# oppo-us-research/PoP-Net

Measured on AMD Instinct MI355X. Metric: depth-frames/sec end-to-end (480x640), higher is better.
Workload: dtype bf16

## Files before the change

popnet_amd/csrc/api.hip:

```cpp
#pragma clang fp contract(off)
#include <cmath>
#include <cstdarg>
#include <cstdio>
#include <cstdlib>
#include <cstring>
#include "pn_internal.h"
#include "preproc_pixel.h"

template <typename TIN>
__global__ void preprocess_kernel(const TIN *__restrict__ depth, float *__restrict__ out, int B, int H, int W, int S,
                                  double scale_x, double scale_y, float dmax, float mean, float stdv) {
    const unsigned pix = blockIdx.x * blockDim.x + threadIdx.x;
    if (pix >= (unsigned)(S * S)) return;
    const int b = blockIdx.y;
    const int dy = (int)(pix / (unsigned)S);
    const int dx = (int)(pix - (unsigned)dy * (unsigned)S);
    const size_t gid = (size_t)b * S * S + pix;

    out[gid] = pn_preproc_pixel(depth + (size_t)b * H * W, H, W, dy, dx, scale_x, scale_y, dmax, mean, stdv);
}

PnSwitches pn_read_switches() {
    auto set = [](const char *name) { return getenv(name) != nullptr; };
    auto num = [](const char *name, int unset) { const char *e = getenv(name); return e ? atoi(e) : unset; };
    auto is = [](const char *name, const char *value) { const char *e = getenv(name); return e && !strcmp(e, value); };
    PnSwitches s;
    s.no_conv3 = set("POPNET_NO_CONV3");
    s.conv3_rpg8 = set("POPNET_CONV3_RPG8");
    s.conv3_pt14 = num("POPNET_CONV3_PT14", 0);
    s.conv3_nbuf2 = set("POPNET_CONV3_NBUF2");
    s.generic_c64_off = num("POPNET_GENERIC_C64", 1) == 0;
    if (set("POPNET_CONV4")) s.conv4 = num("POPNET_CONV4", 0) == 0 ? 0 : 1;
    s.no_mix = set("POPNET_NO_MIX");
    s.no_bblock = set("POPNET_NO_BBLOCK");
    s.bblock_x3 = num("POPNET_BBLOCK_X3", 0) != 0;
    s.bb64_static = set("POPNET_BB64_STATIC");
    s.bb64_halves = num("POPNET_BB64_HALVES", 1) == 2 ? 2 : 1;
    if (set("POPNET_BB64_STRIP")) { const int v = num("POPNET_BB64_STRIP", 0); s.bb64_strip = v == 1 || v == 2 ? v : 0; }
    s.no_tailfuse = set("POPNET_NO_TAILFUSE");
    s.no_poolfuse = set("POPNET_NO_POOLFUSE");
    s.no_stempool = set("POPNET_NO_STEMPOOL");
    s.no_embed3 = set("POPNET_NO_EMBED3");
    s.train_x3_wide = set("POPNET_TRAIN_X3_WIDE");
    s.train_wgrad_novec = set("POPNET_TRAIN_WGRAD_NOVEC");
    s.trainx_one_stream = num("POPNET_TRAINX_STREAMS", 0) == 1;
    s.trainx_stem_handover = set("POPNET_TRAINX_STEM_HANDOVER");
    s.trainx_stem_gather = is("POPNET_TRAINX_STEM_FWD", "gather");
    s.trainx_stem_bn_separate = is("POPNET_TRAINX_STEM_BN", "separate");
    s.trainx_stem_depth = num("POPNET_TRAINX_STEM_DEPTH", 2);
    s.trainx_pack_gather = is("POPNET_TRAINX_PACK", "gather");
    s.trainx_legacy_wgrad = is("POPNET_TRAINX_WGRAD", "legacy");
    return s;
}

extern "C" {

int pn_abi_version(void) { return PN_ABI_VERSION; }
int pn_build_experiments(void) { return 0; }

pn_ctx *pn_create(int device_id) {
    pn_ctx *ctx = new pn_ctx();
    ctx->device = device_id;
    int ndev = 0;
    hipError_t e = hipGetDeviceCount(&ndev);
    if (e != hipSuccess || device_id < 0 || device_id >= ndev) {
        char buf[256];
        snprintf(buf, sizeof buf, "pn_create: device %d not available (%d devices, %s)", device_id, ndev,
                 hipGetErrorString(e));
        ctx->err = buf;
        ctx->device = -1;
        return ctx;
    }
    hipDeviceProp_t prop;
    if (hipGetDeviceProperties(&prop, device_id) == hipSuccess) ctx->num_cus = prop.multiProcessorCount;
    return ctx;
}

void pn_destroy(pn_ctx *ctx) {
    if (!ctx) return;
    if (ctx->parse_ws) (void)hipFree(ctx->parse_ws);
    pn_parse_big_free(ctx);
    if (ctx->train_ws) (void)hipFree(ctx->train_ws);
    for (void *p : ctx->train_ws_retired) (void)hipFree(p);
    for (auto &e : ctx->train_packs) (void)hipFree(e.buf);
    if (ctx->train_pack_table) (void)hipFree(ctx->train_pack_table);
    delete ctx;
}

}

int pn_set_error(pn_ctx *ctx, int code, const char *fmt, ...) {
    char buf[1024];
    va_list ap;
    va_start(ap, fmt);
    vsnprintf(buf, sizeof(buf), fmt, ap);
    va_end(ap);
    if (ctx) ctx->err = buf;
    return code;
}

extern "C" {

int pn_last_error(pn_ctx *ctx, char *buf, size_t buf_len) {
    if (!ctx) return 0;
    if (buf && buf_len) {
        size_t n = ctx->err.size() < buf_len - 1 ? ctx->err.size() : buf_len - 1;
        memcpy(buf, ctx->err.data(), n);
        buf[n] = 0;
    }
    return (int)ctx->err.size();
}

int pn_preprocess(pn_ctx *ctx, const void *depth_dev, int depth_dtype, int B, int H, int W, float *out_dev, int S,
                  float depth_max, float depth_mean, float depth_std, void *hip_stream) {
    if (!ctx) return PN_ERR_INVALID;
    if (ctx->device < 0) return pn_set_error(ctx, PN_ERR_STATE, "context has no device");
    if (!depth_dev || !out_dev || B < 1 || H < 2 || W < 2 || S < 1)
        return pn_set_error(ctx, PN_ERR_INVALID, "pn_preprocess: bad arguments");
    if (W == 2 * S && H == 2 * S)
        return pn_set_error(ctx, PN_ERR_UNSUPPORTED, "pn_preprocess: %dx%d -> %d is an exact 2x decimation, where cv2.resize(INTER_LINEAR) runs INTER_AREA instead: not built", W, H, S);
    const double inv_x = (double)S / (double)W, inv_y = (double)S / (double)H;
    const double scale_x = 1.0 / inv_x, scale_y = 1.0 / inv_y;
    if (B > 65535 || (size_t)S * S > 0x7fffffffu) return pn_set_error(ctx, PN_ERR_INVALID, "pn_preprocess: batch or output size out of range");
    dim3 grid((unsigned)(((size_t)S * S + 255) / 256), (unsigned)B), block(256);
    hipStream_t s = (hipStream_t)hip_stream;
    if (depth_dtype == PN_DEPTH_F16)
        hipLaunchKernelGGL(preprocess_kernel<_Float16>, grid, block, 0, s, (const _Float16 *)depth_dev, out_dev, B, H, W, S,
                           scale_x, scale_y, depth_max, depth_mean, depth_std);
    else if (depth_dtype == PN_DEPTH_F32)
        hipLaunchKernelGGL(preprocess_kernel<float>, grid, block, 0, s, (const float *)depth_dev, out_dev, B, H, W, S,
                           scale_x, scale_y, depth_max, depth_mean, depth_std);
    else
        return pn_set_error(ctx, PN_ERR_INVALID, "pn_preprocess: unknown depth dtype %d", depth_dtype);
    PN_HIP_CHECK(ctx, hipGetLastError());
    return PN_OK;
}

size_t pn_sizeof_parse_cfg(void) { return sizeof(pn_parse_cfg); }

void pn_parse_cfg_default(pn_parse_cfg *cfg) {
    if (!cfg) return;
    cfg->thresh_heatmap = 0.1f;
    cfg->thresh_paf = 0.05f;
    cfg->num_intermed_pts = 10;
    cfg->downsample = 8;
    cfg->input_size = 224;
    cfg->w_org = 480;
    cfg->h_org = 640;
    cfg->fx = 504.1189880371094;
    cfg->fy = 504.042724609375;
    cfg->cx = 231.7421875;
    cfg->cy = 320.62640380859375;
    cfg->depth_mean = 3.f;
    cfg->depth_std = 2.f;
    cfg->z_readout = PN_Z_READOUT_HEAT_WEIGHTED;
    for (int j = 0; j < PN_NUM_JOINTS; ++j) cfg->z_chn[j] = j;
}

}
```

popnet_amd/csrc/conv_misc.hip:

```cpp
#include "pn_internal.h"
#include "preproc_pixel.h"

typedef __attribute__((ext_vector_type(8))) __bf16 bf16x8;
typedef __attribute__((ext_vector_type(4))) float f32x4;

template <typename T>
__global__ __launch_bounds__(256) void stem7x7_kernel(const float *__restrict__ x, const float *__restrict__ w,
                                                       const float *__restrict__ bias, T *__restrict__ out,
                                                       int H, int W, int Ho, int Wo, int out_cs, int split) {
    __shared__ float tile[37][40];
    __shared__ __attribute__((aligned(16))) float wl[49 * 64];
    const int tid = threadIdx.x;
    const int b = blockIdx.z;
    const int oy0 = blockIdx.y * 16, ox0 = blockIdx.x * 16;
    const int iy0 = oy0 * 2 - 3, ix0 = ox0 * 2 - 3;
    for (int i = tid; i < 49 * 64; i += 256) wl[i] = w[i];
    const float *xb = x + (size_t)b * H * W;
    for (int i = tid; i < 37 * 37; i += 256) {
        int r = i / 37, cc = i - r * 37;
        int iy = iy0 + r, ix = ix0 + cc;
        float v = 0.f;
        if ((unsigned)iy < (unsigned)H && (unsigned)ix < (unsigned)W) v = xb[(size_t)iy * W + ix];
        tile[r][cc] = v;
    }
    __syncthreads();
    const int ty = tid >> 4, tx = tid & 15;
    const int oy = oy0 + ty, ox = ox0 + tx;
    float acc[64];
#pragma unroll
    for (int i = 0; i < 64; ++i) acc[i] = 0.f;
    for (int ky = 0; ky < 7; ++ky) {
#pragma unroll
        for (int kx = 0; kx < 7; ++kx) {
            const float xv = tile[ty * 2 + ky][tx * 2 + kx];
            const f32x4 *wp = reinterpret_cast<const f32x4 *>(&wl[(ky * 7 + kx) * 64]);
#pragma unroll
            for (int i = 0; i < 16; ++i) {
                f32x4 w4 = wp[i];
                acc[4 * i + 0] = fmaf(xv, w4[0], acc[4 * i + 0]);
                acc[4 * i + 1] = fmaf(xv, w4[1], acc[4 * i + 1]);
                acc[4 * i + 2] = fmaf(xv, w4[2], acc[4 * i + 2]);
                acc[4 * i + 3] = fmaf(xv, w4[3], acc[4 * i + 3]);
            }
        }
    }
    if (oy < Ho && ox < Wo) {
        T *op = out + ((size_t)(b * Ho + oy) * Wo + ox) * out_cs;
#pragma unroll
        for (int i = 0; i < 64; ++i) {
            float v = acc[i] + bias[i];
            v = v > 0.f ? v : 0.f;
            const T hi = (T)v;
            op[i] = hi;
            if (split) {
                op[split + i] = (T)(v - (float)hi);
            }
        }
    }
}

typedef __attribute__((ext_vector_type(8))) __bf16 stem_bf16x8;
typedef __attribute__((ext_vector_type(4))) unsigned int stem_u32x4;
#define STEM_PITCH 96

template <bool LO>
__device__ __forceinline__ void stem_put(__bf16 *tile, __bf16 *tile_lo, int idx, float v) {
    const __bf16 vh = (__bf16)v;
    tile[idx] = vh;
    if (LO) tile_lo[idx] = (__bf16)(v - (float)vh);
}
template <int ROWS, bool LO>
__device__ __forceinline__ void stem_fill_f32(__bf16 *tile, __bf16 *tile_lo, const float *xb, int iy0, int ix0, int H, int W, int tid) {
    for (int i = tid; i < ROWS * 38; i += 256) {
        const int r = i / 38, cc = i - r * 38;
        const int iy = iy0 + r, ix = ix0 + cc;
        float v = 0.f;
        if (r < ROWS - 1 && (unsigned)iy < (unsigned)H && (unsigned)ix < (unsigned)W) v = xb[(size_t)iy * W + ix];
        stem_put<LO>(tile, tile_lo, r * STEM_PITCH + cc, v);
    }
}
template <int SRC, int ROWS, bool LO>
__device__ __forceinline__ void stem_fill_frames(__bf16 *tile, __bf16 *tile_lo, const PnFrameSrc &src, int b, int iy0, int ix0, int H, int W, int tid) {
    __shared__ PnAxisX axs[38];
    __shared__ PnAxisY ays[ROWS];
    if (tid < 38) axs[tid] = pn_preproc_axis_x(ix0 + tid, src.scale_x, src.W);
    else if (tid >= 64 && tid < 64 + ROWS) ays[tid - 64] = pn_preproc_axis_y(iy0 + tid - 64, src.scale_y, src.H);
    __syncthreads();
    for (int i = tid; i < ROWS * 38; i += 256) {
        const int r = i / 38, cc = i - r * 38;
        const int iy = iy0 + r, ix = ix0 + cc;
        float v = 0.f;
        if (r < ROWS - 1 && (unsigned)iy < (unsigned)H && (unsigned)ix < (unsigned)W) {
            if (SRC == 1) v = pn_preproc_combine((const _Float16 *)src.frames + (size_t)b * src.H * src.W, src.W, axs[cc], ays[r], src.dmax, src.mean, src.stdv);
            else v = pn_preproc_combine((const float *)src.frames + (size_t)b * src.H * src.W, src.W, axs[cc], ays[r], src.dmax, src.mean, src.stdv);
        }
        stem_put<LO>(tile, tile_lo, r * STEM_PITCH + cc, v);
    }
}
template <bool X3> struct StemW { stem_bf16x8 aw[4][2], awl[X3 ? 4 : 1][2]; float bs[16]; };
template <bool X3>
__device__ __forceinline__ void stem_load_w(StemW<X3> &w, const __bf16 *__restrict__ wfrag, const float *__restrict__ bias, int lane, int q) {
#pragma unroll
    for (int t = 0; t < 4; ++t)
#pragma unroll
        for (int s = 0; s < 2; ++s) {
            w.aw[t][s] = *reinterpret_cast<const stem_bf16x8 *>(wfrag + ((t * 2 + s) * 64 + lane) * 8);
            if (X3) w.awl[t][s] = *reinterpret_cast<const stem_bf16x8 *>(wfrag + ((8 + t * 2 + s) * 64 + lane) * 8);
        }
#pragma unroll
    for (int i = 0; i < 16; ++i) w.bs[i] = bias[16 * q + i];
}
template <bool X3>
__device__ __forceinline__ void stem_row(const StemW<X3> &w, const __bf16 *tile, const __bf16 *tile_lo, int ry, int q, int c, f32x4 (&acc)[4]) {
#pragma unroll
    for (int t = 0; t < 4; ++t) acc[t] = f32x4{0.f, 0.f, 0.f, 0.f};
#pragma unroll
    for (int s = 0; s < 2; ++s) {
        const unsigned *src = reinterpret_cast<const unsigned *>(&tile[(2 * ry + 4 * s + q) * STEM_PITCH + 2 * c]);
        stem_u32x4 raw = {src[0], src[1], src[2], src[3]};
        stem_bf16x8 bf = *reinterpret_cast<stem_bf16x8 *>(&raw);
#pragma unroll
        for (int t = 0; t < 4; ++t) acc[t] = __builtin_amdgcn_mfma_f32_16x16x32_bf16(w.aw[t][s], bf, acc[t], 0, 0, 0);
        if (X3) {
            const unsigned *srl = reinterpret_cast<const unsigned *>(&tile_lo[(2 * ry + 4 * s + q) * STEM_PITCH + 2 * c]);
            stem_u32x4 rawl = {srl[0], srl[1], srl[2], srl[3]};
            stem_bf16x8 bl = *reinterpret_cast<stem_bf16x8 *>(&rawl);
#pragma unroll
            for (int t = 0; t < 4; ++t) {
                acc[t] = __builtin_amdgcn_mfma_f32_16x16x32_bf16(w.aw[t][s], bl, acc[t], 0, 0, 0);
                acc[t] = __builtin_amdgcn_mfma_f32_16x16x32_bf16(w.awl[t][s], bf, acc[t], 0, 0, 0);
            }
        }
    }
}
__device__ __forceinline__ void stem_out16(const f32x4 (&acc)[4], const float (&bs)[16], bool lo, __bf16 (&o)[16]) {
#pragma unroll
    for (int t = 0; t < 4; ++t)
#pragma unroll
        for (int r = 0; r < 4; ++r) {
            float v = acc[t][r] + bs[4 * t + r];
            v = v > 0.f ? v : 0.f;
            const __bf16 hi = (__bf16)v;
            o[4 * t + r] = lo ? (__bf16)(v - (float)hi) : hi;
        }
}

template <bool X3, int SRC = 0>
__global__ __launch_bounds__(256) void stem7x7_mfma_kernel(const float *__restrict__ x, const __bf16 *__restrict__ wfrag,
                                                            const float *__restrict__ bias, __bf16 *__restrict__ out,
                                                            int H, int W, int Ho, int Wo, int out_cs, int split, PnFrameSrc src) {
    __shared__ __attribute__((aligned(16))) __bf16 tile[38 * STEM_PITCH];
    __shared__ __attribute__((aligned(16))) __bf16 tile_lo[X3 ? 38 * STEM_PITCH : 8];
    const int tid = threadIdx.x, lane = tid & 63, wave = tid >> 6;
    const int c = lane & 15, q = lane >> 4;
    const int b = blockIdx.z, oy0 = blockIdx.y * 16, ox0 = blockIdx.x * 16;
    const int iy0 = oy0 * 2 - 3, ix0 = ox0 * 2 - 4;
    const float *xb = x + (size_t)b * H * W;
    if (SRC != 0) {
        stem_fill_frames<SRC, 38, X3>(tile, tile_lo, src, b, iy0, ix0, H, W, tid);
    } else if ((W & 3) == 0) {
        for (int i = tid; i < 38 * 10; i += 256) {
            const int r = i / 10, g = i - r * 10;
            const int iy = iy0 + r, ix = ix0 + 4 * g;
            float4 v = {0.f, 0.f, 0.f, 0.f};
            if (r < 37 && (unsigned)iy < (unsigned)H && (unsigned)ix < (unsigned)W) v = *reinterpret_cast<const float4 *>(xb + (size_t)iy * W + ix);
            const float vv[4] = {v.x, v.y, v.z, v.w};
            __bf16 h4[4], l4[4];
#pragma unroll
            for (int k = 0; k < 4; ++k) {
                h4[k] = (__bf16)vv[k];
                l4[k] = (__bf16)(vv[k] - (float)h4[k]);
            }
            *reinterpret_cast<uint2 *>(&tile[r * STEM_PITCH + 4 * g]) = *reinterpret_cast<uint2 *>(h4);
            if (X3) *reinterpret_cast<uint2 *>(&tile_lo[r * STEM_PITCH + 4 * g]) = *reinterpret_cast<uint2 *>(l4);
        }
    } else
        stem_fill_f32<38, X3>(tile, tile_lo, xb, iy0, ix0, H, W, tid);
    StemW<X3> w;
    stem_load_w(w, wfrag, bias, lane, q);
    __syncthreads();
#pragma unroll
    for (int rr = 0; rr < 4; ++rr) {
        const int ry = wave * 4 + rr;
        f32x4 acc[4];
        stem_row(w, tile, tile_lo, ry, q, c, acc);
        const int oy = oy0 + ry, ox = ox0 + c;
        if (oy < Ho && ox < Wo) {
            for (int pl = 0; pl < (split ? 2 : 1); ++pl) {
                __bf16 o[16];
                stem_out16(acc, w.bs, pl == 1, o);
                __bf16 *op = out + ((size_t)(b * Ho + oy) * Wo + ox) * out_cs + 16 * q + pl * split;
                reinterpret_cast<stem_u32x4 *>(op)[0] = reinterpret_cast<stem_u32x4 *>(o)[0];
                reinterpret_cast<stem_u32x4 *>(op)[1] = reinterpret_cast<stem_u32x4 *>(o)[1];
            }
        }
    }
}

template <int SRC>
__global__ __launch_bounds__(256) void stem7x7_pool_kernel(const float *__restrict__ x, const __bf16 *__restrict__ wfrag,
                                                            const float *__restrict__ bias, __bf16 *__restrict__ out,
                                                            int H, int W, int Ho, int Wo, int Hp, int Wp, int out_cs, PnFrameSrc src) {
    __shared__ __attribute__((aligned(16))) __bf16 tile[40 * STEM_PITCH];
    __shared__ __attribute__((aligned(16))) __bf16 otile[17 * 16 * 64];
    const int tid = threadIdx.x, lane = tid & 63, wave = tid >> 6;
    const int c = lane & 15, q = lane >> 4;
    const int b = blockIdx.z, py0 = blockIdx.y * 8, px0 = blockIdx.x * 7;
    const int oy0 = 2 * py0 - 1, ox0 = 2 * px0 - 1;
    const int iy0 = oy0 * 2 - 3, ix0 = ox0 * 2 - 4;
    if (SRC != 0) stem_fill_frames<SRC, 40, false>(tile, nullptr, src, b, iy0, ix0, H, W, tid);
    else stem_fill_f32<40, false>(tile, nullptr, x + (size_t)b * H * W, iy0, ix0, H, W, tid);
    StemW<false> w;
    stem_load_w(w, wfrag, bias, lane, q);
    __syncthreads();
    for (int rr = 0; rr < 5; ++rr) {
        const int ry = wave * 5 + rr;
        if (ry >= 17) break;
        f32x4 acc[4];
        stem_row(w, tile, nullptr, ry, q, c, acc);
        __bf16 o[16];
        stem_out16(acc, w.bs, false, o);
        stem_u32x4 *dst = reinterpret_cast<stem_u32x4 *>(&otile[(ry * 16 + c) * 64 + 16 * q]);
        dst[0] = reinterpret_cast<stem_u32x4 *>(o)[0];
        dst[1] = reinterpret_cast<stem_u32x4 *>(o)[1];
    }
    __syncthreads();
    for (int item = tid; item < 8 * 7 * 8; item += 256) {
        const int g8 = item & 7, pp = item >> 3, pi = pp / 7, pj = pp - pi * 7;
        const int py = py0 + pi, px = px0 + pj;
        if (py >= Hp || px >= Wp) continue;
        float m[8];
#pragma unroll
        for (int k = 0; k < 8; ++k) m[k] = -INFINITY;
#pragma unroll
        for (int ky = 0; ky < 3; ++ky)
#pragma unroll
            for (int kx = 0; kx < 3; ++kx) {
                const int ry = 2 * pi + ky, cc = 2 * pj + kx;
                const bool ok = (unsigned)(oy0 + ry) < (unsigned)Ho && (unsigned)(ox0 + cc) < (unsigned)Wo;
                __bf16 tv[8];
                *reinterpret_cast<stem_u32x4 *>(tv) = *reinterpret_cast<const stem_u32x4 *>(&otile[(ry * 16 + cc) * 64 + g8 * 8]);
#pragma unroll
                for (int k = 0; k < 8; ++k) m[k] = ok ? fmaxf(m[k], (float)tv[k]) : m[k];
            }
        __bf16 o8[8];
#pragma unroll
        for (int k = 0; k < 8; ++k) o8[k] = (__bf16)m[k];
        *reinterpret_cast<stem_u32x4 *>(out + ((size_t)(b * Hp + py) * Wp + px) * out_cs + g8 * 8) = *reinterpret_cast<stem_u32x4 *>(o8);
    }
}

int pn_launch_stem_pool(pn_ctx *ctx, const float *x, const void *wfrag, const float *bias, void *out, int B, int H, int W, int Ho, int Wo,
                        int out_cs, hipStream_t stream, const PnFrameSrc *src) {
    const int Hp = (Ho - 1) / 2 + 1, Wp = (Wo - 1) / 2 + 1;
    dim3 grid((Wp + 6) / 7, (Hp + 7) / 8, B), block(256);
    const PnFrameSrc none = {};
    if (!src) hipLaunchKernelGGL(stem7x7_pool_kernel<0>, grid, block, 0, stream, x, (const __bf16 *)wfrag, bias, (__bf16 *)out, H, W, Ho, Wo, Hp, Wp, out_cs, none);
    else if (src->dtype == PN_DEPTH_F16) hipLaunchKernelGGL(stem7x7_pool_kernel<1>, grid, block, 0, stream, x, (const __bf16 *)wfrag, bias, (__bf16 *)out, H, W, Ho, Wo, Hp, Wp, out_cs, *src);
    else hipLaunchKernelGGL(stem7x7_pool_kernel<2>, grid, block, 0, stream, x, (const __bf16 *)wfrag, bias, (__bf16 *)out, H, W, Ho, Wo, Hp, Wp, out_cs, *src);
    PN_HIP_CHECK(ctx, hipGetLastError());
    return PN_OK;
}

int pn_launch_stem(pn_ctx *ctx, int prec, const float *x, const float *w, const void *wfrag, const float *bias, void *out,
                   int B, int H, int W, int Ho, int Wo, int out_cs, int split, hipStream_t stream, const PnFrameSrc *src) {
    dim3 grid((Wo + 15) / 16, (Ho + 15) / 16, B), block(256);
    const PnFrameSrc none = {};
    if (src) {
        const bool f16 = src->dtype == PN_DEPTH_F16;
        if (prec == PN_PREC_BF16 && f16) hipLaunchKernelGGL((stem7x7_mfma_kernel<false, 1>), grid, block, 0, stream, x, (const __bf16 *)wfrag, bias, (__bf16 *)out, H, W, Ho, Wo, out_cs, split, *src);
        else if (prec == PN_PREC_BF16) hipLaunchKernelGGL((stem7x7_mfma_kernel<false, 2>), grid, block, 0, stream, x, (const __bf16 *)wfrag, bias, (__bf16 *)out, H, W, Ho, Wo, out_cs, split, *src);
        else if (prec == PN_PREC_BF16X3 && f16) hipLaunchKernelGGL((stem7x7_mfma_kernel<true, 1>), grid, block, 0, stream, x, (const __bf16 *)wfrag, bias, (__bf16 *)out, H, W, Ho, Wo, out_cs, split, *src);
        else if (prec == PN_PREC_BF16X3) hipLaunchKernelGGL((stem7x7_mfma_kernel<true, 2>), grid, block, 0, stream, x, (const __bf16 *)wfrag, bias, (__bf16 *)out, H, W, Ho, Wo, out_cs, split, *src);
        else return pn_set_error(ctx, PN_ERR_UNSUPPORTED, "the frames-in stem is built for the bf16 and bf16x3 nets");
        PN_HIP_CHECK(ctx, hipGetLastError());
        return PN_OK;
    }
    if (prec == PN_PREC_BF16)
        hipLaunchKernelGGL((stem7x7_mfma_kernel<false, 0>), grid, block, 0, stream, x, (const __bf16 *)wfrag, bias, (__bf16 *)out, H, W, Ho, Wo, out_cs, split, none);
    else if (prec == PN_PREC_BF16X3)
        hipLaunchKernelGGL((stem7x7_mfma_kernel<true, 0>), grid, block, 0, stream, x, (const __bf16 *)wfrag, bias, (__bf16 *)out, H, W, Ho, Wo, out_cs, split, none);
    else
        hipLaunchKernelGGL(stem7x7_kernel<float>, grid, block, 0, stream, x, w, bias, (float *)out, H, W, Ho, Wo, out_cs, 0);
    PN_HIP_CHECK(ctx, hipGetLastError());
    return PN_OK;
}

template <typename T, int MODE, bool SPLIT = false>
__global__ void pool_kernel(const T *__restrict__ in, T *__restrict__ out, int B, int H, int W, int Ho, int Wo,
                            int C8, int in_cs, int out_cs, int out_coff, int in_split, int out_split) {
    size_t gid = (size_t)blockIdx.x * blockDim.x + threadIdx.x;
    size_t total = (size_t)B * Ho * Wo * C8;
    if (gid >= total) return;
    int c8 = (int)(gid % C8);
    size_t p = gid / C8;
    int ox = (int)(p % Wo);
    size_t t = p / Wo;
    int oy = (int)(t % Ho);
    int b = (int)(t / Ho);
    constexpr int K = (MODE == 2) ? 2 : 3;
    constexpr int PAD = (MODE == 2) ? 0 : 1;
    float acc[8];
#pragma unroll
    for (int i = 0; i < 8; ++i) acc[i] = (MODE == 0) ? 0.f : -INFINITY;
    T v[K * K][8], v2[K * K][8];
    bool ok[K * K];
#pragma unroll
    for (int ky = 0; ky < K; ++ky)
#pragma unroll
        for (int kx = 0; kx < K; ++kx) {
            const int iy = oy * 2 - PAD + ky, ix = ox * 2 - PAD + kx;
            ok[ky * K + kx] = (unsigned)iy < (unsigned)H && (unsigned)ix < (unsigned)W;
            const int cy = min(max(iy, 0), H - 1), cx = min(max(ix, 0), W - 1);
            const T *ip = in + ((size_t)(b * H + cy) * W + cx) * in_cs + c8 * 8;
            if (sizeof(T) == 2) {
                *reinterpret_cast<uint4 *>(v[ky * K + kx]) = *reinterpret_cast<const uint4 *>(ip);
                if (SPLIT) *reinterpret_cast<uint4 *>(v2[ky * K + kx]) = *reinterpret_cast<const uint4 *>(ip + in_split);
            } else {
                reinterpret_cast<uint4 *>(v[ky * K + kx])[0] = reinterpret_cast<const uint4 *>(ip)[0];
                reinterpret_cast<uint4 *>(v[ky * K + kx])[1] = reinterpret_cast<const uint4 *>(ip)[1];
            }
        }
#pragma unroll
    for (int k = 0; k < K * K; ++k) {
        float f[8];
#pragma unroll
        for (int i = 0; i < 8; ++i) f[i] = (float)v[k][i];
        if (sizeof(T) == 2 && SPLIT) {
#pragma unroll
            for (int i = 0; i < 8; ++i) f[i] += (float)v2[k][i];
        }
#pragma unroll
        for (int i = 0; i < 8; ++i) {
            if (MODE == 0) acc[i] += ok[k] ? f[i] : 0.f;
            else acc[i] = ok[k] ? fmaxf(acc[i], f[i]) : acc[i];
        }
    }
    for (int pl = 0; pl < (out_split ? 2 : 1); ++pl) {
        T o[8];
#pragma unroll
        for (int i = 0; i < 8; ++i) {
            const float r = (MODE == 0) ? acc[i] / 9.0f : acc[i];
            const T hi = (T)r;
            o[i] = pl == 1 ? (T)(r - (float)hi) : hi;
        }
        T *op = out + p * out_cs + out_coff + c8 * 8 + pl * out_split;
        if (sizeof(T) == 2) {
            *reinterpret_cast<uint4 *>(op) = *reinterpret_cast<uint4 *>(o);
        } else {
            reinterpret_cast<uint4 *>(op)[0] = reinterpret_cast<uint4 *>(o)[0];
            reinterpret_cast<uint4 *>(op)[1] = reinterpret_cast<uint4 *>(o)[1];
        }
    }
}

template <typename T>
static void launch_pool_t(int mode, const void *in, void *out, int B, int H, int W, int Ho, int Wo, int C,
                          int in_cs, int out_cs, int out_coff, int in_split, int out_split, hipStream_t stream) {
    size_t total = (size_t)B * Ho * Wo * (C / 8);
    dim3 grid((unsigned)((total + 255) / 256)), block(256);
    if (sizeof(T) == 2 && in_split) {
        if (mode == 0)
            hipLaunchKernelGGL((pool_kernel<T, 0, true>), grid, block, 0, stream, (const T *)in, (T *)out, B, H, W, Ho, Wo, C / 8, in_cs, out_cs, out_coff, in_split, out_split);
        else if (mode == 1)
            hipLaunchKernelGGL((pool_kernel<T, 1, true>), grid, block, 0, stream, (const T *)in, (T *)out, B, H, W, Ho, Wo, C / 8, in_cs, out_cs, out_coff, in_split, out_split);
        else
            hipLaunchKernelGGL((pool_kernel<T, 2, true>), grid, block, 0, stream, (const T *)in, (T *)out, B, H, W, Ho, Wo, C / 8, in_cs, out_cs, out_coff, in_split, out_split);
        return;
    }
    if (mode == 0)
        hipLaunchKernelGGL((pool_kernel<T, 0>), grid, block, 0, stream, (const T *)in, (T *)out, B, H, W, Ho, Wo, C / 8, in_cs, out_cs, out_coff, in_split, out_split);
    else if (mode == 1)
        hipLaunchKernelGGL((pool_kernel<T, 1>), grid, block, 0, stream, (const T *)in, (T *)out, B, H, W, Ho, Wo, C / 8, in_cs, out_cs, out_coff, in_split, out_split);
    else
// ... 70 lines not shown
```

popnet_amd/csrc/net_api.hip:

```cpp
#include <cstdarg>
#include <cstdio>
#include <cstring>
#include "net_internal.h"

using namespace pnnet;

namespace {
std::string geom_json(int prec, bool x3, const ConvGeom &g, int H, int W, int cout, int cin_chunks, int B) {
    ConvProblem P;
    memset(&P, 0, sizeof P);
    pn_fill_conv_problem(P, {nullptr, H, W, 0, 64, 0}, B, cin_chunks, cout, g, prec, x3);
    char t[384];
    snprintf(t, sizeof t, "\"kernel\": \"%s\", \"kern\": %d, \"cfg\": %d, \"pitch\": %d, \"R\": %d, \"Wt\": %d, \"wc\": %d, \"wp\": %d, \"nbuf\": %d, \"pt\": %d, \"rpg\": %d, "
             "\"tiles_x\": %d, \"tiles_per_img\": %d, \"cout_blocks\": %d, \"nblocks\": %d, \"lds_two\": %d",
             (g.dil != 1 ? pn_conv_kernel_label_dil(prec, g.ks, g.stride, g.pitch, g.cfg, g.dil) : pn_conv_kernel_label(prec, g.kern, false, g.ks, g.stride, g.pitch, g.cfg, g.wc, g.wp, g.nbuf, g.pt, g.rpg)).c_str(), g.kern, g.cfg, g.pitch, g.R, g.Wt, g.wc,
             g.wp, g.nbuf, g.pt, g.rpg, P.tiles_x, P.tiles_per_img, P.cout_blocks, P.nblocks, P.lds_two);
    return t;
}

int forward_entry(pn_net *n, int kind, bool pointers_ok, bool state = true) {
    if (!n) return PN_ERR_INVALID;
    pn_ctx *ctx = n->ctx;
    if (n->kind != kind)
        return pn_set_error(ctx, PN_ERR_INVALID, "not %s net", kind == PN_NET_RTPOSE_LIGHT3D ? "an rtpose_light3d" : kind == PN_NET_YOLO_POSENET ? "a YoloPoseNet" : "an A2J");
    if (!pointers_ok) return pn_set_error(ctx, PN_ERR_INVALID, "null device pointer");
    if (state && ctx->device < 0) return pn_set_error(ctx, PN_ERR_STATE, "context has no device");
    if (state && !n->finalized) return pn_set_error(ctx, PN_ERR_STATE, "pn_net_finalize has not been called");
    return PN_OK;
}

int forward_frames(pn_net *n, const void *depth_dev, int depth_dtype, int B, int H, int W, float depth_max, float depth_mean, float depth_std,
                   hipStream_t stream, int nsteps = -1, bool partial = false) {
    pn_ctx *ctx = n->ctx;
    if (!depth_dev || H < 2 || W < 2) return pn_set_error(ctx, PN_ERR_INVALID, "forward_frames: bad arguments");
    if (depth_dtype != PN_DEPTH_F16 && depth_dtype != PN_DEPTH_F32) return pn_set_error(ctx, PN_ERR_INVALID, "forward_frames: unknown depth dtype %d", depth_dtype);
    if (int rc = forward_entry(n, n->kind, true)) return rc;
    if (n->prec != PN_PREC_BF16) return pn_set_error(ctx, PN_ERR_UNSUPPORTED, "the frames-in forward is built for the bf16 and bf16x3 nets (fp32: pn_preprocess + pn_*_forward)");
    if (n->in_h != n->in_w) return pn_set_error(ctx, PN_ERR_UNSUPPORTED, "the frames-in forward resizes to a square input (net finalized for %dx%d)", n->in_h, n->in_w);
    const int S = n->in_h;
    if (W == 2 * S && H == 2 * S)
        return pn_set_error(ctx, PN_ERR_UNSUPPORTED, "forward_frames: %dx%d -> %d is an exact 2x decimation, where cv2.resize(INTER_LINEAR) runs INTER_AREA instead: not built", W, H, S);
    if (partial) {
        if (n->last_B < 0) return pn_set_error(ctx, PN_ERR_STATE, "pn_net_forward_frames_partial: run one full forward first");
        if (nsteps < 0 || nsteps > (int)n->steps.size()) return pn_set_error(ctx, PN_ERR_INVALID, "nsteps %d outside [0, %zu]", nsteps, n->steps.size());
    }
    PnFrameSrc fs;
    fs.frames = depth_dev; fs.dtype = depth_dtype; fs.H = H; fs.W = W;
    const double inv_x = (double)S / (double)W, inv_y = (double)S / (double)H;
    fs.scale_x = 1.0 / inv_x; fs.scale_y = 1.0 / inv_y;
    fs.dmax = depth_max; fs.mean = depth_mean; fs.stdv = depth_std;
    n->frame_src = fs;
    const int rc = run_forward(n, nullptr, B, stream, nsteps);
    n->frame_src.frames = nullptr;
    return rc;
}
}

extern "C" {
pn_net *pn_net_create(pn_ctx *ctx, int kind, int num_parts, int a, int input_dim) {
    if (!ctx) return nullptr;
    if (kind != PN_NET_RTPOSE_LIGHT3D && kind != PN_NET_YOLO_POSENET && kind != PN_NET_A2J) {
        pn_set_error(ctx, PN_ERR_INVALID, "unknown net kind %d", kind);
        return nullptr;
    }
    if (input_dim < 1 || input_dim > 16) {
        pn_set_error(ctx, PN_ERR_UNSUPPORTED, "input_dim %d outside [1, 16]", input_dim);
        return nullptr;
    }
    if (kind == PN_NET_A2J && input_dim != 1) {
        pn_set_error(ctx, PN_ERR_UNSUPPORTED, "the A2J net takes one-channel depth crops (input_dim = 1)");
        return nullptr;
    }
    pn_net *n = new pn_net();
    n->ctx = ctx; n->kind = kind; n->num_parts = num_parts; n->a = a; n->input_dim = input_dim;
    return n;
}

void pn_net_destroy(pn_net *n) {
    if (!n) return;
    release_net(n);
    delete n;
}

int pn_net_set_tensor(pn_net *n, const char *name, const float *host_data, const int64_t *shape, int ndim) {
    if (!n || !name || (!host_data && ndim > 0)) return PN_ERR_INVALID;
    if (n->finalized) return pn_set_error(n->ctx, PN_ERR_STATE, "net already finalized");
    std::string s(name);
    if (s.rfind("module.", 0) == 0) s = s.substr(7);
    if (n->kind == PN_NET_A2J && (s.rfind("Backbone.model.fc.", 0) == 0 || (s.size() > 19 && s.compare(s.size() - 19, 19, "num_batches_tracked") == 0)))
        return PN_OK;
    HostTensor t;
    size_t numel = 1;
    for (int i = 0; i < ndim; ++i) { t.shape.push_back(shape[i]); numel *= (size_t)shape[i]; }
    t.data.assign(host_data, host_data + numel);
    n->tensors[s] = std::move(t);
    return PN_OK;
}

int pn_net_finalize(pn_net *n, int precision, int max_batch, int in_h, int in_w) {
    if (!n) return PN_ERR_INVALID;
    pn_ctx *ctx = n->ctx;
    if (n->finalized) return pn_set_error(ctx, PN_ERR_STATE, "net already finalized");
    if (precision != PN_PREC_F32 && precision != PN_PREC_BF16 && precision != PN_PREC_BF16X3) return pn_set_error(ctx, PN_ERR_INVALID, "bad precision %d", precision);
    if (max_batch < 1) return pn_set_error(ctx, PN_ERR_INVALID, "max_batch must be >= 1");
    n->x3 = precision == PN_PREC_BF16X3;
    n->prec = n->x3 ? PN_PREC_BF16 : precision; n->max_batch = max_batch; n->in_h = in_h; n->in_w = in_w;
    n->sw = pn_read_switches();
    if (int rc = compile_net(n)) return rc;
    if (ctx->device >= 0)
        if (int rc = upload_net(n)) return rc;
    for (auto &im : n->images) std::vector<unsigned char>().swap(im.host);
    n->tensors.clear();
    n->finalized = true;
    return PN_OK;
}

int pn_rtpose_forward(pn_net *n, const float *x_dev, int B, float *paf_dev, float *heat_dev, float *z_dev, void *hip_stream) {
    if (int rc = forward_entry(n, PN_NET_RTPOSE_LIGHT3D, x_dev && paf_dev && heat_dev && z_dev)) return rc;
    n->nchw_ptr[0] = paf_dev; n->nchw_ptr[1] = heat_dev; n->nchw_ptr[2] = z_dev;
    return run_forward(n, x_dev, B, (hipStream_t)hip_stream);
}

int pn_yolo_forward(pn_net *n, const float *x_dev, int B, float *out_dev, void *hip_stream) {
    if (int rc = forward_entry(n, PN_NET_YOLO_POSENET, x_dev && out_dev)) return rc;
    n->nchw_ptr[3] = out_dev;
    return run_forward(n, x_dev, B, (hipStream_t)hip_stream);
}

int pn_a2j_forward(pn_net *n, const float *crops_dev, int B, const void **cls_dev, const void **reg_dev, const void **dep_dev, void *hip_stream) {
    if (int rc = forward_entry(n, PN_NET_A2J, crops_dev != nullptr)) return rc;
    if (int rc = run_forward(n, crops_dev, B, (hipStream_t)hip_stream)) return rc;
    if (cls_dev) *cls_dev = n->bufs[n->named["cls"].buf].p;
    if (reg_dev) *reg_dev = n->bufs[n->named["reg"].buf].p;
    if (dep_dev) *dep_dev = n->bufs[n->named["dep"].buf].p;
    return PN_OK;
}

int pn_a2j_head_shape(pn_net *n, int *h, int *w, int *precision) {
    if (!n) return PN_ERR_INVALID;
    if (n->kind != PN_NET_A2J || !n->finalized) return pn_set_error(n->ctx, PN_ERR_STATE, "not a finalized A2J net");
    if (h) *h = n->out_h;
    if (w) *w = n->out_w;
    if (precision) *precision = n->x3 ? PN_PREC_BF16X3 : n->prec;
    return PN_OK;
}

int pn_a2j_predict(pn_net *n, const void *frames_dev, int depth_dtype, int F, int H, int W, const float *rows_dev, int nrows, const pn_a2j_cfg *cfg,
                   const float *anchors_dev, float *crops_dev, int32_t *flags_dev, float *votes_dev, pn_a2j_record *records_dev, void *hip_stream) {
    if (!n) return PN_ERR_INVALID;
    pn_ctx *ctx = n->ctx;
    if (n->kind != PN_NET_A2J || !n->finalized) return pn_set_error(ctx, PN_ERR_STATE, "not a finalized A2J net");
    if (ctx->device < 0) return pn_set_error(ctx, PN_ERR_STATE, "context has no device");
    if (!cfg || !crops_dev || !anchors_dev) return pn_set_error(ctx, PN_ERR_INVALID, "pn_a2j_predict: null argument");
    if (cfg->crop_h != n->in_h || cfg->crop_w != n->in_w)
        return pn_set_error(ctx, PN_ERR_INVALID, "pn_a2j_predict: crops of %dx%d into a net finalized for %dx%d", cfg->crop_h, cfg->crop_w, n->in_h, n->in_w);
    if (nrows < 1 || nrows > n->max_batch) return pn_set_error(ctx, PN_ERR_INVALID, "pn_a2j_predict: %d rows outside [1, %d]", nrows, n->max_batch);
    if (int rc = pn_a2j_crop(ctx, frames_dev, depth_dtype, F, H, W, rows_dev, nrows, cfg, crops_dev, flags_dev, hip_stream)) return rc;
    const void *cls = nullptr, *reg = nullptr, *dep = nullptr;
    if (int rc = pn_a2j_forward(n, crops_dev, nrows, &cls, &reg, &dep, hip_stream)) return rc;
    return pn_a2j_vote(ctx, cls, reg, dep, n->x3 ? PN_PREC_BF16X3 : n->prec, nrows, n->out_h, n->out_w, 16, n->num_parts, anchors_dev, votes_dev, rows_dev, cfg, records_dev, hip_stream);
}

int pn_rtpose_forward_frames(pn_net *n, const void *depth_dev, int depth_dtype, int B, int H, int W, float depth_max, float depth_mean, float depth_std,
                             float *paf_dev, float *heat_dev, float *z_dev, void *hip_stream) {
    if (int rc = forward_entry(n, PN_NET_RTPOSE_LIGHT3D, paf_dev && heat_dev && z_dev, false)) return rc;
    n->nchw_ptr[0] = paf_dev; n->nchw_ptr[1] = heat_dev; n->nchw_ptr[2] = z_dev;
    return forward_frames(n, depth_dev, depth_dtype, B, H, W, depth_max, depth_mean, depth_std, (hipStream_t)hip_stream);
}

int pn_yolo_forward_frames(pn_net *n, const void *depth_dev, int depth_dtype, int B, int H, int W, float depth_max, float depth_mean, float depth_std,
                           float *out_dev, void *hip_stream) {
    if (int rc = forward_entry(n, PN_NET_YOLO_POSENET, out_dev != nullptr, false)) return rc;
    n->nchw_ptr[3] = out_dev;
    return forward_frames(n, depth_dev, depth_dtype, B, H, W, depth_max, depth_mean, depth_std, (hipStream_t)hip_stream);
}

int pn_net_copy_activation(pn_net *n, const char *name, int B, float *dev_out, void *hip_stream) {
    if (!n || !name || !dev_out) return PN_ERR_INVALID;
    pn_ctx *ctx = n->ctx;
    if (ctx->device < 0) return pn_set_error(ctx, PN_ERR_STATE, "context has no device");
    if (!n->finalized) return pn_set_error(ctx, PN_ERR_STATE, "net not finalized");
    auto it = n->named.find(name);
    if (it == n->named.end()) return pn_set_error(ctx, PN_ERR_INVALID, "unknown activation '%s'", name);
    const NamedAct &a = it->second;
    const Buf &b = n->bufs[a.buf];
    const bool one = a.plane >= 0;
    return pn_launch_nhwc_to_nchw(ctx, n->prec, b.p, dev_out, B, b.H, b.W, a.C, b.C, a.coff + (one ? a.plane * b.plane : 0), n->x3 && !one ? b.plane : 0, (hipStream_t)hip_stream);
}

int pn_net_read_activation(pn_net *n, const char *name, int B, float *host_out, size_t host_elems, void *hip_stream) {
    if (!n || !name || !host_out) return PN_ERR_INVALID;
    pn_ctx *ctx = n->ctx;
    if (ctx->device < 0) return pn_set_error(ctx, PN_ERR_STATE, "context has no device");
    auto it = n->named.find(name);
    if (it == n->named.end()) return pn_set_error(ctx, PN_ERR_INVALID, "unknown activation '%s'", name);
    const Buf &b = n->bufs[it->second.buf];
    const size_t elems = (size_t)B * it->second.C * b.H * b.W;
    if (host_elems < elems) return pn_set_error(ctx, PN_ERR_INVALID, "host buffer too small: %zu < %zu", host_elems, elems);
    float *tmp = nullptr;
    PN_HIP_CHECK(ctx, hipMalloc((void **)&tmp, elems * 4));
    hipStream_t s = (hipStream_t)hip_stream;
    int rc = pn_net_copy_activation(n, name, B, tmp, hip_stream);
    if (!rc) {
// ... 149 lines not shown
```

popnet_amd/csrc/preproc_pixel.h:

```cpp
#pragma once

struct PnFrameSrc {
    const void *frames;
    int dtype;
    int H, W;
    double scale_x, scale_y;
    float dmax, mean, stdv;
};

struct PnAxisX { int sx; float fx; };
struct PnAxisY { int y0, y1; float fy; };

__device__ __forceinline__ PnAxisX pn_preproc_axis_x(int dx, double scale_x, int W) {
#pragma clang fp contract(off)
    float fx = (float)(((double)dx + 0.5) * scale_x - 0.5);
    int sx = (int)floorf(fx);
    fx -= (float)sx;
    if (sx < 0) { sx = 0; fx = 0.f; }
    if (sx >= W - 1) { sx = W - 1; fx = 0.f; }
    return PnAxisX{sx, fx};
}

__device__ __forceinline__ PnAxisY pn_preproc_axis_y(int dy, double scale_y, int H) {
#pragma clang fp contract(off)
    float fy = (float)(((double)dy + 0.5) * scale_y - 0.5);
    const int sy = (int)floorf(fy);
    fy -= (float)sy;
    return PnAxisY{min(max(sy, 0), H - 1), min(max(sy + 1, 0), H - 1), fy};
}

template <typename TIN>
__device__ __forceinline__ float pn_preproc_combine(const TIN *__restrict__ img, int W, PnAxisX ax, PnAxisY ay, float dmax, float mean, float stdv) {
#pragma clang fp contract(off)
    const float a0 = 1.f - ax.fx, a1 = ax.fx;
    float h0, h1;
    if (ax.sx + 1 >= W) {
        h0 = (float)img[(size_t)ay.y0 * W + ax.sx];
        h1 = (float)img[(size_t)ay.y1 * W + ax.sx];
    } else {
        h0 = (float)img[(size_t)ay.y0 * W + ax.sx] * a0 + (float)img[(size_t)ay.y0 * W + ax.sx + 1] * a1;
        h1 = (float)img[(size_t)ay.y1 * W + ax.sx] * a0 + (float)img[(size_t)ay.y1 * W + ax.sx + 1] * a1;
    }
    float v = h0 * (1.f - ay.fy) + h1 * ay.fy;
    if (v < 0.f) v = 0.f;
    if (v > dmax) v = dmax;
    return (v - mean) / stdv;
}

template <typename TIN>
__device__ __forceinline__ float pn_preproc_pixel(const TIN *__restrict__ img, int H, int W, int dy, int dx, double scale_x, double scale_y,
                                                  float dmax, float mean, float stdv) {
    return pn_preproc_combine(img, W, pn_preproc_axis_x(dx, scale_x, W), pn_preproc_axis_y(dy, scale_y, H), dmax, mean, stdv);
}
```

Measured before the change: 69630.

## Restructure frames-in stem fill with per-thread column pairs and exact reciprocal normalization

Rewrites the frames-in stem tile fill so each thread owns two adjacent columns across 13-row strides. Row byte offsets are precomputed in shared memory, tail handling is hoisted out of the loop, and the two values go to LDS with one paired bf16 store. Division by the depth std is replaced by multiplication with an exact power-of-two reciprocal when std is a power of two, which keeps the result bit-identical. The stem epilogue is also specialized at compile time for the lo/hi split, and the output address is hoisted. The cost is 32-bit offset math, which needs a new guard that rejects frames of 2^29 pixels or more.

```diff
diff --git a/popnet_amd/csrc/api.hip b/popnet_amd/csrc/api.hip
--- a/popnet_amd/csrc/api.hip
+++ b/popnet_amd/csrc/api.hip
@@ -9,7 +9,7 @@
 
 template <typename TIN>
 __global__ void preprocess_kernel(const TIN *__restrict__ depth, float *__restrict__ out, int B, int H, int W, int S,
-                                  double scale_x, double scale_y, float dmax, float mean, float stdv) {
+                                  double scale_x, double scale_y, float dmax, float mean, float stdv, float rstd) {
     const unsigned pix = blockIdx.x * blockDim.x + threadIdx.x;
     if (pix >= (unsigned)(S * S)) return;
     const int b = blockIdx.y;
@@ -17,7 +17,7 @@
     const int dx = (int)(pix - (unsigned)dy * (unsigned)S);
     const size_t gid = (size_t)b * S * S + pix;
 
-    out[gid] = pn_preproc_pixel(depth + (size_t)b * H * W, H, W, dy, dx, scale_x, scale_y, dmax, mean, stdv);
+    out[gid] = pn_preproc_pixel(depth + (size_t)b * H * W, H, W, dy, dx, scale_x, scale_y, dmax, mean, stdv, rstd);
 }
 
 PnSwitches pn_read_switches() {
@@ -124,12 +124,13 @@
     if (B > 65535 || (size_t)S * S > 0x7fffffffu) return pn_set_error(ctx, PN_ERR_INVALID, "pn_preprocess: batch or output size out of range");
     dim3 grid((unsigned)(((size_t)S * S + 255) / 256), (unsigned)B), block(256);
     hipStream_t s = (hipStream_t)hip_stream;
+    const float rstd = pn_preproc_rstd(depth_std);
     if (depth_dtype == PN_DEPTH_F16)
         hipLaunchKernelGGL(preprocess_kernel<_Float16>, grid, block, 0, s, (const _Float16 *)depth_dev, out_dev, B, H, W, S,
-                           scale_x, scale_y, depth_max, depth_mean, depth_std);
+                           scale_x, scale_y, depth_max, depth_mean, depth_std, rstd);
     else if (depth_dtype == PN_DEPTH_F32)
         hipLaunchKernelGGL(preprocess_kernel<float>, grid, block, 0, s, (const float *)depth_dev, out_dev, B, H, W, S,
-                           scale_x, scale_y, depth_max, depth_mean, depth_std);
+                           scale_x, scale_y, depth_max, depth_mean, depth_std, rstd);
     else
         return pn_set_error(ctx, PN_ERR_INVALID, "pn_preprocess: unknown depth dtype %d", depth_dtype);
     PN_HIP_CHECK(ctx, hipGetLastError());
diff --git a/popnet_amd/csrc/conv_misc.hip b/popnet_amd/csrc/conv_misc.hip
--- a/popnet_amd/csrc/conv_misc.hip
+++ b/popnet_amd/csrc/conv_misc.hip
@@ -1,5 +1,6 @@
 #include "pn_internal.h"
 #include "preproc_pixel.h"
+#include <type_traits>
 
 typedef __attribute__((ext_vector_type(8))) __bf16 bf16x8;
 typedef __attribute__((ext_vector_type(4))) float f32x4;
@@ -69,6 +70,13 @@
     tile[idx] = vh;
     if (LO) tile_lo[idx] = (__bf16)(v - (float)vh);
 }
+template <bool LO>
+__device__ __forceinline__ void stem_put2(__bf16 *tile, __bf16 *tile_lo, int idx, float v0, float v1) {
+    typedef __attribute__((ext_vector_type(2))) __bf16 bf16x2;
+    const bf16x2 vh = {(__bf16)v0, (__bf16)v1};
+    *reinterpret_cast<bf16x2 *>(&tile[idx]) = vh;
+    if (LO) *reinterpret_cast<bf16x2 *>(&tile_lo[idx]) = bf16x2{(__bf16)(v0 - (float)vh[0]), (__bf16)(v1 - (float)vh[1])};
+}
 template <int ROWS, bool LO>
 __device__ __forceinline__ void stem_fill_f32(__bf16 *tile, __bf16 *tile_lo, const float *xb, int iy0, int ix0, int H, int W, int tid) {
     for (int i = tid; i < ROWS * 38; i += 256) {
@@ -79,22 +87,61 @@
         stem_put<LO>(tile, tile_lo, r * STEM_PITCH + cc, v);
     }
 }
+struct StemRowY { unsigned off0, off1; float fy; int ok; };
+template <typename TIN, int ROWS, bool LO, bool NOTAIL>
+__device__ __forceinline__ void stem_fill_rows(__bf16 *tile, __bf16 *tile_lo, const char *__restrict__ fb, const StemRowY *ays, const PnFrameSrc &src,
+                                               int r, int cc, const unsigned (&sxb)[2], const float (&a0)[2], const float (&a1)[2], const bool (&tail)[2], const bool (&okx)[2]) {
+    for (; r < ROWS; r += 13) {
+        const StemRowY ay = ays[r];
+        float v[2];
+#pragma unroll
+        for (int j = 0; j < 2; ++j) {
+            const bool t = NOTAIL ? false : tail[j];
+            const float h0 = pn_preproc_h(reinterpret_cast<const TIN *>(fb + (ay.off0 + sxb[j])), t, a0[j], a1[j]);
+            const float h1 = pn_preproc_h(reinterpret_cast<const TIN *>(fb + (ay.off1 + sxb[j])), t, a0[j], a1[j]);
+            v[j] = pn_preproc_v(h0, h1, ay.fy, src.dmax, src.mean);
+        }
+        if (src.rstd != 0.f) {
+            v[0] = pn_preproc_norm(v[0], src.stdv, src.rstd);
+            v[1] = pn_preproc_norm(v[1], src.stdv, src.rstd);
+        } else {
+            v[0] = pn_preproc_norm(v[0], src.stdv, 0.f);
+            v[1] = pn_preproc_norm(v[1], src.stdv, 0.f);
+        }
+        v[0] = ay.ok && okx[0] ? v[0] : 0.f;
+        v[1] = ay.ok && okx[1] ? v[1] : 0.f;
+        stem_put2<LO>(tile, tile_lo, r * STEM_PITCH + cc, v[0], v[1]);
+    }
+}
 template <int SRC, int ROWS, bool LO>
 __device__ __forceinline__ void stem_fill_frames(__bf16 *tile, __bf16 *tile_lo, const PnFrameSrc &src, int b, int iy0, int ix0, int H, int W, int tid) {
+    typedef typename std::conditional<SRC == 1, _Float16, float>::type TIN;
     __shared__ PnAxisX axs[38];
-    __shared__ PnAxisY ays[ROWS];
+    __shared__ StemRowY ays[ROWS];
     if (tid < 38) axs[tid] = pn_preproc_axis_x(ix0 + tid, src.scale_x, src.W);
-    else if (tid >= 64 && tid < 64 + ROWS) ays[tid - 64] = pn_preproc_axis_y(iy0 + tid - 64, src.scale_y, src.H);
+    else if (tid >= 64 && tid < 64 + ROWS) {
+        const int r = tid - 64;
+        const PnAxisY ay = pn_preproc_axis_y(iy0 + r, src.scale_y, src.H);
+        ays[r] = StemRowY{(unsigned)(ay.y0 * src.W) * (unsigned)sizeof(TIN), (unsigned)(ay.y1 * src.W) * (unsigned)sizeof(TIN), ay.fy,
+                          r < ROWS - 1 && (unsigned)(iy0 + r) < (unsigned)H};
+    }
     __syncthreads();
-    for (int i = tid; i < ROWS * 38; i += 256) {
-        const int r = i / 38, cc = i - r * 38;
-        const int iy = iy0 + r, ix = ix0 + cc;
-        float v = 0.f;
-        if (r < ROWS - 1 && (unsigned)iy < (unsigned)H && (unsigned)ix < (unsigned)W) {
-            if (SRC == 1) v = pn_preproc_combine((const _Float16 *)src.frames + (size_t)b * src.H * src.W, src.W, axs[cc], ays[r], src.dmax, src.mean, src.stdv);
-            else v = pn_preproc_combine((const float *)src.frames + (size_t)b * src.H * src.W, src.W, axs[cc], ays[r], src.dmax, src.mean, src.stdv);
-        }
-        stem_put<LO>(tile, tile_lo, r * STEM_PITCH + cc, v);
+    const int rp = tid / 19, cc = 2 * (tid - 19 * rp);
+    if (rp < 13) {
+        const char *fb = reinterpret_cast<const char *>(src.frames) + (size_t)b * src.H * src.W * sizeof(TIN);
+        unsigned sxb[2];
+        float a0[2], a1[2];
+        bool tail[2], okx[2];
+#pragma unroll
+        for (int j = 0; j < 2; ++j) {
+            const PnAxisX ax = axs[cc + j];
+            sxb[j] = (unsigned)ax.sx * (unsigned)sizeof(TIN);
+            a0[j] = 1.f - ax.fx; a1[j] = ax.fx;
+            tail[j] = ax.sx + 1 >= src.W;
+            okx[j] = (unsigned)(ix0 + cc + j) < (unsigned)W;
+        }
+        if (tail[0] || tail[1]) stem_fill_rows<TIN, ROWS, LO, false>(tile, tile_lo, fb, ays, src, rp, cc, sxb, a0, a1, tail, okx);
+        else stem_fill_rows<TIN, ROWS, LO, true>(tile, tile_lo, fb, ays, src, rp, cc, sxb, a0, a1, tail, okx);
     }
 }
 template <bool X3> struct StemW { stem_bf16x8 aw[4][2], awl[X3 ? 4 : 1][2]; float bs[16]; };
@@ -133,15 +180,20 @@
         }
     }
 }
-__device__ __forceinline__ void stem_out16(const f32x4 (&acc)[4], const float (&bs)[16], bool lo, __bf16 (&o)[16]) {
+template <bool LO>
+__device__ __forceinline__ void stem_out16(const f32x4 (&acc)[4], const float (&bs)[16], __bf16 (&o)[16]) {
+    typedef __attribute__((ext_vector_type(2))) float f32x2;
 #pragma unroll
     for (int t = 0; t < 4; ++t)
 #pragma unroll
-        for (int r = 0; r < 4; ++r) {
-            float v = acc[t][r] + bs[4 * t + r];
-            v = v > 0.f ? v : 0.f;
-            const __bf16 hi = (__bf16)v;
-            o[4 * t + r] = lo ? (__bf16)(v - (float)hi) : hi;
+        for (int r = 0; r < 4; r += 2) {
+            f32x2 v = f32x2{acc[t][r], acc[t][r + 1]} + f32x2{bs[4 * t + r], bs[4 * t + r + 1]};
+#pragma unroll
+            for (int k = 0; k < 2; ++k) {
+                v[k] = v[k] > 0.f ? v[k] : 0.f;
+                const __bf16 hi = (__bf16)v[k];
+                o[4 * t + r + k] = LO ? (__bf16)(v[k] - (float)hi) : hi;
+            }
         }
 }
 
@@ -179,19 +231,24 @@
     StemW<X3> w;
     stem_load_w(w, wfrag, bias, lane, q);
     __syncthreads();
+    const int ox = ox0 + c;
+    const size_t o0 = ((size_t)(b * Ho + oy0 + wave * 4) * Wo + ox) * out_cs + 16 * q, orow = (size_t)Wo * out_cs;
 #pragma unroll
     for (int rr = 0; rr < 4; ++rr) {
         const int ry = wave * 4 + rr;
         f32x4 acc[4];
         stem_row(w, tile, tile_lo, ry, q, c, acc);
-        const int oy = oy0 + ry, ox = ox0 + c;
+        const int oy = oy0 + ry;
         if (oy < Ho && ox < Wo) {
-            for (int pl = 0; pl < (split ? 2 : 1); ++pl) {
-                __bf16 o[16];
-                stem_out16(acc, w.bs, pl == 1, o);
-                __bf16 *op = out + ((size_t)(b * Ho + oy) * Wo + ox) * out_cs + 16 * q + pl * split;
-                reinterpret_cast<stem_u32x4 *>(op)[0] = reinterpret_cast<stem_u32x4 *>(o)[0];
-                reinterpret_cast<stem_u32x4 *>(op)[1] = reinterpret_cast<stem_u32x4 *>(o)[1];
+            __bf16 *op = out + (o0 + rr * orow);
+            __bf16 o[16];
+            stem_out16<false>(acc, w.bs, o);
+            reinterpret_cast<stem_u32x4 *>(op)[0] = reinterpret_cast<stem_u32x4 *>(o)[0];
+            reinterpret_cast<stem_u32x4 *>(op)[1] = reinterpret_cast<stem_u32x4 *>(o)[1];
+            if (X3) {
+                stem_out16<true>(acc, w.bs, o);
+                reinterpret_cast<stem_u32x4 *>(op + split)[0] = reinterpret_cast<stem_u32x4 *>(o)[0];
+                reinterpret_cast<stem_u32x4 *>(op + split)[1] = reinterpret_cast<stem_u32x4 *>(o)[1];
             }
         }
     }
@@ -219,7 +276,7 @@
         f32x4 acc[4];
         stem_row(w, tile, nullptr, ry, q, c, acc);
         __bf16 o[16];
-        stem_out16(acc, w.bs, false, o);
+        stem_out16<false>(acc, w.bs, o);
         stem_u32x4 *dst = reinterpret_cast<stem_u32x4 *>(&otile[(ry * 16 + c) * 64 + 16 * q]);
         dst[0] = reinterpret_cast<stem_u32x4 *>(o)[0];
         dst[1] = reinterpret_cast<stem_u32x4 *>(o)[1];
diff --git a/popnet_amd/csrc/net_api.hip b/popnet_amd/csrc/net_api.hip
--- a/popnet_amd/csrc/net_api.hip
+++ b/popnet_amd/csrc/net_api.hip
@@ -34,6 +34,8 @@
     pn_ctx *ctx = n->ctx;
     if (!depth_dev || H < 2 || W < 2) return pn_set_error(ctx, PN_ERR_INVALID, "forward_frames: bad arguments");
     if (depth_dtype != PN_DEPTH_F16 && depth_dtype != PN_DEPTH_F32) return pn_set_error(ctx, PN_ERR_INVALID, "forward_frames: unknown depth dtype %d", depth_dtype);
+    if ((long long)H * W >= (1ll << 29))
+        return pn_set_error(ctx, PN_ERR_UNSUPPORTED, "forward_frames: a %dx%d frame is beyond the 2^29 pixels the frames-in stem addresses (pn_preprocess + pn_*_forward)", W, H);
     if (int rc = forward_entry(n, n->kind, true)) return rc;
     if (n->prec != PN_PREC_BF16) return pn_set_error(ctx, PN_ERR_UNSUPPORTED, "the frames-in forward is built for the bf16 and bf16x3 nets (fp32: pn_preprocess + pn_*_forward)");
     if (n->in_h != n->in_w) return pn_set_error(ctx, PN_ERR_UNSUPPORTED, "the frames-in forward resizes to a square input (net finalized for %dx%d)", n->in_h, n->in_w);
@@ -49,6 +51,7 @@
     const double inv_x = (double)S / (double)W, inv_y = (double)S / (double)H;
     fs.scale_x = 1.0 / inv_x; fs.scale_y = 1.0 / inv_y;
     fs.dmax = depth_max; fs.mean = depth_mean; fs.stdv = depth_std;
+    fs.rstd = pn_preproc_rstd(depth_std);
     n->frame_src = fs;
     const int rc = run_forward(n, nullptr, B, stream, nsteps);
     n->frame_src.frames = nullptr;
diff --git a/popnet_amd/csrc/preproc_pixel.h b/popnet_amd/csrc/preproc_pixel.h
--- a/popnet_amd/csrc/preproc_pixel.h
+++ b/popnet_amd/csrc/preproc_pixel.h
@@ -1,4 +1,5 @@
 #pragma once
+#include <cmath>
 
 struct PnFrameSrc {
     const void *frames;
@@ -6,7 +7,14 @@
     int H, W;
     double scale_x, scale_y;
     float dmax, mean, stdv;
+    float rstd;
 };
+
+inline float pn_preproc_rstd(float stdv) {
+    int e = 0;
+    if (!(stdv > 0.f) || frexpf(stdv, &e) != 0.5f || e < -63 || e > 65) return 0.f;
+    return ldexpf(1.f, 1 - e);
+}
 
 struct PnAxisX { int sx; float fx; };
 struct PnAxisY { int y0, y1; float fy; };
@@ -30,25 +38,37 @@
 }
 
 template <typename TIN>
-__device__ __forceinline__ float pn_preproc_combine(const TIN *__restrict__ img, int W, PnAxisX ax, PnAxisY ay, float dmax, float mean, float stdv) {
+__device__ __forceinline__ float pn_preproc_h(const TIN *__restrict__ p, bool tail, float a0, float a1) {
+#pragma clang fp contract(off)
+    if (tail) return (float)p[0];
+    return (float)p[0] * a0 + (float)p[1] * a1;
+}
+
+__device__ __forceinline__ float pn_preproc_v(float h0, float h1, float fy, float dmax, float mean) {
+#pragma clang fp contract(off)
+    float v = h0 * (1.f - fy) + h1 * fy;
+    if (v < 0.f) v = 0.f;
+    if (v > dmax) v = dmax;
+    return v - mean;
+}
+
+__device__ __forceinline__ float pn_preproc_norm(float d, float stdv, float rstd) {
+#pragma clang fp contract(off)
+    return rstd != 0.f ? d * rstd : d / stdv;
+}
+
+template <typename TIN>
+__device__ __forceinline__ float pn_preproc_combine(const TIN *__restrict__ img, int W, PnAxisX ax, PnAxisY ay, float dmax, float mean, float stdv, float rstd) {
 #pragma clang fp contract(off)
     const float a0 = 1.f - ax.fx, a1 = ax.fx;
-    float h0, h1;
-    if (ax.sx + 1 >= W) {
-        h0 = (float)img[(size_t)ay.y0 * W + ax.sx];
-        h1 = (float)img[(size_t)ay.y1 * W + ax.sx];
-    } else {
-        h0 = (float)img[(size_t)ay.y0 * W + ax.sx] * a0 + (float)img[(size_t)ay.y0 * W + ax.sx + 1] * a1;
-        h1 = (float)img[(size_t)ay.y1 * W + ax.sx] * a0 + (float)img[(size_t)ay.y1 * W + ax.sx + 1] * a1;
-    }
-    float v = h0 * (1.f - ay.fy) + h1 * ay.fy;
-    if (v < 0.f) v = 0.f;
-    if (v > dmax) v = dmax;
-    return (v - mean) / stdv;
+    const bool tail = ax.sx + 1 >= W;
+    const float h0 = pn_preproc_h(img + (size_t)ay.y0 * W + ax.sx, tail, a0, a1);
+    const float h1 = pn_preproc_h(img + (size_t)ay.y1 * W + ax.sx, tail, a0, a1);
+    return pn_preproc_norm(pn_preproc_v(h0, h1, ay.fy, dmax, mean), stdv, rstd);
 }
 
 template <typename TIN>
 __device__ __forceinline__ float pn_preproc_pixel(const TIN *__restrict__ img, int H, int W, int dy, int dx, double scale_x, double scale_y,
-                                                  float dmax, float mean, float stdv) {
-    return pn_preproc_combine(img, W, pn_preproc_axis_x(dx, scale_x, W), pn_preproc_axis_y(dy, scale_y, H), dmax, mean, stdv);
+                                                  float dmax, float mean, float stdv, float rstd = 0.f) {
+    return pn_preproc_combine(img, W, pn_preproc_axis_x(dx, scale_x, W), pn_preproc_axis_y(dy, scale_y, H), dmax, mean, stdv, rstd);
 }
```

New measurement: 69580. About the same (-0.1%).
